# haan6/fm-for-online-recommendation

Measured on AMD Instinct MI355X. Metric: samples/sec online-FM (Criteo-39-field, k=16) FTRL-proximal, higher is better.
Workload: dtype f32

## Files before the change

fm-for-online-recommendation_amd/csrc/fmx_common.h:

```cpp
#pragma once
#include <hip/hip_runtime.h>
#include <hip/hip_ext.h>

#include <cstdarg>
#include <cstdio>
#include <cstdlib>
#include <cstring>
#include <atomic>
#include <mutex>

#include "fmx.h"

#pragma clang fp contract(off)

namespace fmxd {
extern thread_local char g_err[512];
int fail(int code, const char *fmt, ...);
int check_launch(const char *what);

struct Tune {
  int wpb_fwd = 2, wpb_upd = 2;
  int sort_e = 0;
  int inline_fixup = 1;
  int online_persistent = 1;
  int sort_ahead = 16;
  int mlp_chain = 1;
  int sort_chunked = 1;
};
Tune &tune();

constexpr int FMX_COMM_SLOTS = 4;
struct Comm {
  int rank = 0, world = 1, n_blocks = 1;
  bool force = false;
  int block_count[FMX_COMM_MAX_WORLD] = {0}, block_first[FMX_COMM_MAX_WORLD] = {0};
  void *main = nullptr, *pf = nullptr;
  hipStream_t pf_stream = nullptr;
  hipEvent_t fork = nullptr, ready[FMX_COMM_SLOTS] = {nullptr}, free_[FMX_COMM_SLOTS] = {nullptr};
  bool used[FMX_COMM_SLOTS] = {false};
};
int comm_all_gather(Comm *c, int which, const void *send, void *recv, size_t count, hipStream_t st);
int comm_exchange_blocks(Comm *c, const float *send, float *recv, size_t per, hipStream_t st);

constexpr int MLP_BIG_MAX_L = 8;
struct MlpReduceArgs {
  const float *parts[MLP_BIG_MAX_L];
  int out_dim[MLP_BIG_MAX_L], in_dim[MLP_BIG_MAX_L], ldp[MLP_BIG_MAX_L];
  long long grad_off[MLP_BIG_MAX_L];
  float *grads;
  float *params;
  float lr;
  int rule;
  float *m, *v;
  float eps, c1, c2;
  int n_split[MLP_BIG_MAX_L], n_layers;
  const float *loss_b;
  float *loss_out;
  int B;
  float inv_b;
};
int mlp_section_deferred_reduce(const fmx_mlp_t *mlp, int32_t loss_kind, const float *bi, int32_t ld_bi, const float *base, const float *y, int32_t B,
                                float inv_b, void *workspace, float *logit_out, float *dz_out, float *gbi_out, int32_t ld_gbi, float *grads,
                                float lr_apply, float *loss_out, hipStream_t st, MlpReduceArgs *deferred, const char *who = "fmx_mlp_section");
void mlp_launch_reduce(const MlpReduceArgs &a, hipStream_t st);
int mlp_opt_check(const fmx_mlp_t *mlp, int32_t B, const void *workspace, int64_t workspace_bytes, const float *grads, const fmx_mlp_opt_t *opt,
                  int64_t n_steps, const char *who);
int mlp_opt_state_check(const fmx_mlp_opt_t *opt, int64_t n_steps, const char *who);
int mlp_reduce_blocks_per_layer(const MlpReduceArgs &a, int threads);
int step_geometry_check(const fmx_table_t *table, int32_t B, const char *who);
}
using namespace fmxd;

namespace {

inline bool aligned16(const void *p) { return (reinterpret_cast<uintptr_t>(p) & 15u) == 0; }

constexpr uint32_t SENT = 0xFFFFFFFFu;
constexpr int WAVE = 64;
constexpr int MAX_SORT_WIDTH = 32768;


__device__ __forceinline__ float4 operator+(float4 a, float4 b) { return {a.x + b.x, a.y + b.y, a.z + b.z, a.w + b.w}; }
__device__ __forceinline__ float4 operator-(float4 a, float4 b) { return {a.x - b.x, a.y - b.y, a.z - b.z, a.w - b.w}; }
__device__ __forceinline__ float4 operator*(float4 a, float4 b) { return {a.x * b.x, a.y * b.y, a.z * b.z, a.w * b.w}; }
__device__ __forceinline__ float4 operator*(float a, float4 b) { return {a * b.x, a * b.y, a * b.z, a * b.w}; }
__device__ __forceinline__ float4 splat(float a) { return {a, a, a, a}; }

__device__ __forceinline__ float4 shfl_xor4(float4 v, int m) {
  return {__shfl_xor(v.x, m), __shfl_xor(v.y, m), __shfl_xor(v.z, m), __shfl_xor(v.w, m)};
}
__device__ __forceinline__ float4 shfl_up4(float4 v, int d) {
  return {__shfl_up(v.x, d), __shfl_up(v.y, d), __shfl_up(v.z, d), __shfl_up(v.w, d)};
}
__device__ __forceinline__ float4 shfl4(float4 v, int src) {
  return {__shfl(v.x, src), __shfl(v.y, src), __shfl(v.z, src), __shfl(v.w, src)};
}

__device__ __forceinline__ float rcp_(float x) { return __builtin_amdgcn_rcpf(x); }
__device__ __forceinline__ float sqrt_(float x) { return __builtin_amdgcn_sqrtf(x); }

__device__ __forceinline__ float ftrl_w(float z, float n, const fmx_hyper_t &h) {
  const float denom = fmaf(h.beta + sqrt_(n), h.alpha, h.l2);
  const float w = -(z - copysignf(h.l1, z)) * rcp_(denom);
  return fabsf(z) <= h.l1 ? 0.f : w;
}
__device__ __forceinline__ float4 ftrl_w4(float4 z, float4 n, const fmx_hyper_t &h) {
  return {ftrl_w(z.x, n.x, h), ftrl_w(z.y, n.y, h), ftrl_w(z.z, n.z, h), ftrl_w(z.w, n.w, h)};
}
__device__ __forceinline__ void ftrl_upd(float &z, float &n, float w, float g, const fmx_hyper_t &h) {
  const float n2 = fmaf(g, g, n);
  const float sigma = (sqrt_(n2) - sqrt_(n)) * h.alpha;
  z = fmaf(-sigma, w, z + g);
  n = n2;
}

template <int RULE>
__device__ __forceinline__ float apply_rule(float p, float g, const fmx_hyper_t &h) {
  if (RULE == FMX_RULE_SIGNADAM) return p - h.lr * g * rcp_(fabsf(g) + h.eps);
  return p - h.lr * g;
}
template <int RULE>
__device__ __forceinline__ float4 apply_rule4(float4 p, float4 g, const fmx_hyper_t &h) {
  return {apply_rule<RULE>(p.x, g.x, h), apply_rule<RULE>(p.y, g.y, h), apply_rule<RULE>(p.z, g.z, h),
          apply_rule<RULE>(p.w, g.w, h)};
}

__host__ __device__ inline double pow_step(double b, int32_t t) {
  double r = 1.0, p = b;
  for (uint32_t e = (uint32_t)t; e; e >>= 1) {
    if (e & 1u) r = r * p;
    p = p * p;
  }
  return r;
}
__host__ __device__ inline void adam_consts(float lr, float beta1, float beta2, int32_t t, float &step_size, float &c1, float &c2,
                                            float eps = 0.f, float *eps_dense = nullptr) {
  const double b1 = beta1, b2 = beta2;
  const double s2 = sqrt(1.0 - pow_step(b2, t));
  step_size = (float)((double)lr * s2 / (1.0 - pow_step(b1, t)));
  c1 = (float)(1.0 - b1);
  c2 = (float)(1.0 - b2);
  if (eps_dense) *eps_dense = (float)((double)eps * s2);
}
template <int RULE>
__device__ __forceinline__ void moments_upd(float &p, float &m, float &v, float g, const fmx_hyper_t &h) {
  if (RULE == FMX_RULE_ADAM) {
    m = m + h.beta1 * (g - m);
    v = v + h.beta2 * (g * g - v);
    p = p - h.lr * (m * rcp_(sqrt_(v) + h.eps));
  } else {
    v = v + g * g;
    p = p - h.lr * (g * rcp_(sqrt_(v) + h.eps));
  }
}
template <int RULE>
__device__ __forceinline__ void moments_upd4(float4 &p, float4 &m, float4 &v, float4 g, const fmx_hyper_t &h) {
  moments_upd<RULE>(p.x, m.x, v.x, g.x, h);
  moments_upd<RULE>(p.y, m.y, v.y, g.y, h);
  moments_upd<RULE>(p.z, m.z, v.z, g.z, h);
  moments_upd<RULE>(p.w, m.w, v.w, g.w, h);
}

template <int LAYOUT>
__device__ __forceinline__ float bias_weight(float b0, float b1, const fmx_hyper_t &h) {
  return LAYOUT == FMX_LAYOUT_FTRL ? ftrl_w(b0, b1, h) : b0;
}
template <int LAYOUT, int RULE>
__device__ __forceinline__ void bias_step(float &b0, float &b1, float &b2, float g, const fmx_hyper_t &h) {
  if (LAYOUT == FMX_LAYOUT_WEIGHTS) {
    b0 = apply_rule<RULE>(b0, g, h);
  } else if (LAYOUT == FMX_LAYOUT_MOMENTS) {
    moments_upd<RULE>(b0, b1, b2, g, h);
  } else {
    const float w = ftrl_w(b0, b1, h);
    ftrl_upd(b0, b1, w, g, h);
  }
}

__device__ __forceinline__ float sigmoidf_(float z) { return 1.f / (1.f + expf(-z)); }
__device__ __forceinline__ float bcewl(float z, float y) {
  return (1.f - y) * z + log1pf(expf(-fabsf(z))) + fmaxf(-z, 0.f);
}
__device__ __forceinline__ void bce_loss_dz(int loss_kind, float z, float y, float inv_b, float &loss, float &dz) {
  if (loss_kind == FMX_LOSS_BCE_LOGITS) {
    loss = bcewl(z, y);
    dz = (sigmoidf_(z) - y) * inv_b;
  } else {
    const float p = sigmoidf_(z);
    loss = bcewl(p, y);
    dz = (sigmoidf_(p) - y) * p * (1.f - p) * inv_b;
  }
}

template <int M>
__device__ __forceinline__ uint32_t xor_lane(uint32_t v, int lane) {
  if constexpr (M == 1) {
    return (uint32_t)__builtin_amdgcn_mov_dpp((int)v, 0xB1, 0xF, 0xF, true);
  } else if constexpr (M == 2) {
    return (uint32_t)__builtin_amdgcn_mov_dpp((int)v, 0x4E, 0xF, 0xF, true);
  } else if constexpr (M == 4) {
    const int t = __builtin_amdgcn_mov_dpp((int)v, 0x141, 0xF, 0xF, true);
    return (uint32_t)__builtin_amdgcn_mov_dpp(t, 0x1B, 0xF, 0xF, true);
  } else if constexpr (M == 8) {
    return (uint32_t)__builtin_amdgcn_mov_dpp((int)v, 0x128, 0xF, 0xF, true);
  } else if constexpr (M == 16) {
    const auto sw = __builtin_amdgcn_permlane16_swap(v, v, false, false);
    return (lane & 16) ? sw[0] : sw[1];
  } else {
    const auto sw = __builtin_amdgcn_permlane32_swap(v, v, false, false);
    return (lane & 32) ? sw[0] : sw[1];
  }
}

template <int M>
__device__ __forceinline__ float xor_lane_f(float v, int lane) {
  return __uint_as_float(xor_lane<M>(__float_as_uint(v), lane));
}
template <int M>
__device__ __forceinline__ float4 xor_lane_f4(float4 v, int lane) {
  return {xor_lane_f<M>(v.x, lane), xor_lane_f<M>(v.y, lane), xor_lane_f<M>(v.z, lane), xor_lane_f<M>(v.w, lane)};
}

template <int M, int LPR>
__device__ __forceinline__ void fm_sums_level(float4 &s, float4 &ss, float &fo, int lane, int groups) {
  if (LPR <= M && M / LPR < groups) {
    s = s + xor_lane_f4<M>(s, lane);
    ss = ss + xor_lane_f4<M>(ss, lane);
    fo += xor_lane_f<M>(fo, lane);
  }
}
template <int LPR>
__device__ __forceinline__ void fm_field_sums(float4 &s, float4 &ss, float &fo, int lane, int groups = WAVE) {
  fm_sums_level<1, LPR>(s, ss, fo, lane, groups);
  fm_sums_level<2, LPR>(s, ss, fo, lane, groups);
  fm_sums_level<4, LPR>(s, ss, fo, lane, groups);
  fm_sums_level<8, LPR>(s, ss, fo, lane, groups);
  fm_sums_level<16, LPR>(s, ss, fo, lane, groups);
  fm_sums_level<32, LPR>(s, ss, fo, lane, groups);
}
template <int LPR>
__device__ __forceinline__ float4 fm_bi(float4 s, float4 ss, float &sbi) {
  const float4 bi = 0.5f * (s * s - ss);
  sbi = (bi.x + bi.y) + (bi.z + bi.w);
#pragma unroll
  for (int m = 1; m < LPR; m <<= 1) sbi += __shfl_xor(sbi, m);
  return bi;
}

__device__ float block_sum(const float *src, int n, int ld, float *sm) {
  constexpr int U = 16;
  const int tid = threadIdx.x, nt = blockDim.x < 128 ? blockDim.x : 128;
  float acc = 0.f;
  if (tid >= nt) {
    __syncthreads();
    for (int w = nt >> 1; w > 0; w >>= 1) __syncthreads();
    const float r = sm[0];
    __syncthreads();
    return r;
  }
  if (ld == 1) {
    const int n4 = n >> 2;
    const float4 *src4 = reinterpret_cast<const float4 *>(src);
    for (int i0 = tid; i0 < n4; i0 += U * nt) {
      float4 v[U];
#pragma unroll
      for (int u = 0; u < U; ++u) {
        const int i = i0 + u * nt;
        v[u] = src4[i < n4 ? i : 0];
      }
#pragma unroll
      for (int u = 0; u < U; ++u) {
        const bool in = i0 + u * nt < n4;
        acc += in ? (v[u].x + v[u].y) + (v[u].z + v[u].w) : 0.f;
      }
    }
    for (int i = (n4 << 2) + tid; i < n; i += nt) acc += src[i];
  } else {
    constexpr int V = 4;
    const int n4 = n >> 2;
    for (int i0 = tid; i0 < n4; i0 += V * nt) {
      float4 v[V];
#pragma unroll
      for (int u = 0; u < V; ++u) {
        const int i = i0 + u * nt;
        const float *p = src + (size_t)(4 * (i < n4 ? i : 0)) * ld;
        v[u] = float4{p[0], p[ld], p[2 * (size_t)ld], p[3 * (size_t)ld]};
      }
#pragma unroll
      for (int u = 0; u < V; ++u) {
        const bool in = i0 + u * nt < n4;
        acc += in ? (v[u].x + v[u].y) + (v[u].z + v[u].w) : 0.f;
      }
    }
    for (int i = (n4 << 2) + tid; i < n; i += nt) acc += src[(size_t)i * ld];
  }
  sm[tid] = acc;
  __syncthreads();
  for (int w = nt >> 1; w > 0; w >>= 1) {
    if (tid < w) sm[tid] += sm[tid + w];
    __syncthreads();
  }
  const float r = sm[0];
  __syncthreads();
  return r;
}

inline size_t align_up(size_t x, size_t a) { return (x + a - 1) / a * a; }

inline void mlp_reduce_set_opt(MlpReduceArgs &a, const fmx_mlp_opt_t &o, int32_t t) {
  a.rule = o.rule;
  a.m = o.m;
  a.v = o.v;
  a.lr = o.lr;
  a.eps = o.eps;
  a.c1 = a.c2 = 0.f;
  if (o.rule == FMX_RULE_ADAM) adam_consts(o.lr, o.beta1, o.beta2, t, a.lr, a.c1, a.c2, o.eps, &a.eps);
}

__device__ __forceinline__ void mlp_reduce_block(const MlpReduceArgs &a, int l, int block, int n_blocks) {
  const int out = a.out_dim[l], in = a.in_dim[l], ldp = a.ldp[l], ns = a.n_split[l];
  const int groups = ldp >> 2;
  const long long n = (long long)out * groups;
  const float *p = a.parts[l];
  const size_t zs = (size_t)out * ldp;
  const bool adaptive = a.rule != FMX_RULE_SGD, apply = adaptive || a.lr != 0.f;
  fmx_hyper_t h;
  h.lr = a.lr;
  h.eps = a.eps;
  h.beta1 = a.c1;
  h.beta2 = a.c2;
  for (long long i = (long long)block * blockDim.x + threadIdx.x; i < n; i += (long long)n_blocks * blockDim.x) {
    const int m = (int)(i / groups), c = (int)(i - (long long)m * groups) * 4;
    const float *q = p + (size_t)m * ldp + c;
    const bool vec4 = apply && c + 3 < in && (in & 3) == 0 && (a.grad_off[l] & 3) == 0;
    float4 pv = {0.f, 0.f, 0.f, 0.f}, mv = pv, vv = pv;
    if (vec4) {
      const long long o = a.grad_off[l] + (long long)m * in + c;
      pv = *reinterpret_cast<const float4 *>(a.params + o);
      if (adaptive) vv = *reinterpret_cast<const float4 *>(a.v + o);
      if (a.rule == FMX_RULE_ADAM) mv = *reinterpret_cast<const float4 *>(a.m + o);
    }
    float4 s = {0.f, 0.f, 0.f, 0.f};
    for (int z0 = 0; z0 < ns; z0 += 16) {
      float4 r[16];
#pragma unroll
      for (int z = 0; z < 16; ++z)
        if (z0 + z < ns) r[z] = *reinterpret_cast<const float4 *>(q + (size_t)(z0 + z) * zs);
#pragma unroll
      for (int z = 0; z < 16; ++z)
        if (z0 + z < ns) {
          s.x += r[z].x;
          s.y += r[z].y;
          s.z += r[z].z;
          s.w += r[z].w;
        }
    }
    if (vec4) {
      const long long o = a.grad_off[l] + (long long)m * in + c;
      *reinterpret_cast<float4 *>(a.grads + o) = s;
      if (a.rule == FMX_RULE_ADAM) {
        moments_upd4<FMX_RULE_ADAM>(pv, mv, vv, s, h);
        *reinterpret_cast<float4 *>(a.m + o) = mv;
        *reinterpret_cast<float4 *>(a.v + o) = vv;
      } else if (adaptive) {
        moments_upd4<FMX_RULE_ADAGRAD>(pv, mv, vv, s, h);
        *reinterpret_cast<float4 *>(a.v + o) = vv;
      } else {
        pv = float4{pv.x - a.lr * s.x, pv.y - a.lr * s.y, pv.z - a.lr * s.z, pv.w - a.lr * s.w};
      }
      *reinterpret_cast<float4 *>(a.params + o) = pv;
      continue;
    }
    const float v[4] = {s.x, s.y, s.z, s.w};
#pragma unroll
    for (int j = 0; j < 4; ++j) {
      if (c + j > in) break;
      const long long o = c + j < in ? a.grad_off[l] + (long long)m * in + c + j : a.grad_off[l] + (long long)out * in + m;
      a.grads[o] = v[j];
      if (!apply) continue;
      if (!adaptive) {
        a.params[o] -= a.lr * v[j];
      } else if (a.rule == FMX_RULE_ADAM) {
        moments_upd<FMX_RULE_ADAM>(a.params[o], a.m[o], a.v[o], v[j], h);
      } else {
        float unused = 0.f;
        moments_upd<FMX_RULE_ADAGRAD>(a.params[o], unused, a.v[o], v[j], h);
      }
    }
  }
  if (block == 0 && l == 0 && a.loss_out) {
    __shared__ float sm[256];
    const float ls = block_sum(a.loss_b, a.B, 1, sm);
    if (threadIdx.x == 0) a.loss_out[0] = ls * a.inv_b;
  }
}

}
```

fm-for-online-recommendation_amd/csrc/fmx_kernels.hip:

```cpp

#include <type_traits>

#include "fmx_common.h"

namespace fmxd {

thread_local char g_err[512] = "";

int fail(int code, const char *fmt, ...) {
  va_list ap;
  va_start(ap, fmt);
  vsnprintf(g_err, sizeof(g_err), fmt, ap);
  va_end(ap);
  return code;
}

int check_launch(const char *what) {
  hipError_t e = hipGetLastError();
  if (e != hipSuccess) return fail(FMX_ERR_LAUNCH, "%s: %s", what, hipGetErrorString(e));
  return FMX_OK;
}

}

namespace {

#include "fmx_sort.inc"

__device__ __forceinline__ void st_sc1(float *p, float v) { __hip_atomic_store(p, v, __ATOMIC_RELAXED, __HIP_MEMORY_SCOPE_AGENT); }
__device__ __forceinline__ float ld_sc1(const float *p) {
  return __hip_atomic_load(p, __ATOMIC_RELAXED, __HIP_MEMORY_SCOPE_AGENT);
}
__device__ __forceinline__ float4 ld_sc1_4(const float *p) { return {ld_sc1(p), ld_sc1(p + 1), ld_sc1(p + 2), ld_sc1(p + 3)}; }
typedef float v4f __attribute__((ext_vector_type(4)));
__device__ __forceinline__ void st_sc1_4(float *p, float4 v) {
  const v4f x = {v.x, v.y, v.z, v.w};
  asm volatile("global_store_dwordx4 %0, %1, off sc1\n\ts_nop 1" ::"v"(p), "v"(x) : "memory");
}
__device__ __forceinline__ void store_part_sc1(float *rec, int q, int kp, float4 cV, float4 cA, float cw) {
  st_sc1_4(rec + 4 * q, cV);
  st_sc1_4(rec + kp + 4 * q, cA);
  if (q == 0) st_sc1(rec + 2 * kp, cw);
}

struct FwdArgs {
  const float *rows;
  const int64_t *foff;
  const float *bias;
  const int32_t *idx;
  const float *xv;
  const float *y;
  fmx_fwd_out_t out;
  fmx_hyper_t h;
  int32_t B, F, kp, stride, zoff, loss_kind;
  int32_t ldS, ld1;
  float inv_b;
  const int32_t *fcols, *fbase;
  int32_t Fc;
};

#ifdef FMX_STAMPS
__device__ unsigned long long g_fwd_stamps[8192 * 6];
#define FMX_FSTAMP(slot_, dep_)                                                                                     \
  do {                                                                                                              \
    unsigned long long t_;                                                                                          \
    asm volatile("s_memrealtime %0\n\ts_waitcnt lgkmcnt(0)" : "=s"(t_) : "v"(dep_) : "memory");                      \
    if (lane == 0 && b < 8192) g_fwd_stamps[(size_t)b * 6 + (slot_)] = t_;                                           \
  } while (0)
#else
#define FMX_FSTAMP(slot_, dep_) do {} while (0)
#endif

template <int LPR>
__device__ __forceinline__ void forward_finish(const FwdArgs &a, const int b, const int lane, float4 s, float4 ss, float fo, bool bad,
                                               const float y_early, const float bias) {
  const int q = lane % LPR;
  const int kp = LPR * 4;
  if (bad && a.out.error) *a.out.error = 1;

  fm_field_sums<LPR>(s, ss, fo, lane);
  float sbi;
  const float4 bi = fm_bi<LPR>(s, ss, sbi);
  fo = __shfl(fo, 0);
  FMX_FSTAMP(3, sbi);

  if (lane < LPR) {
    if (a.out.S) *reinterpret_cast<float4 *>(a.out.S + (size_t)b * a.ldS + 4 * q) = s;
    if (a.out.bi) *reinterpret_cast<float4 *>(a.out.bi + (size_t)b * kp + 4 * q) = bi;
  }
  if (lane == 0) {
    const float z = fo + sbi + bias;
    if (a.out.sfirst) a.out.sfirst[b] = fo;
    if (a.out.sbi) a.out.sbi[b] = sbi;
    if (a.out.logit) a.out.logit[b] = z;
    if (a.loss_kind != FMX_LOSS_NONE) {
      float loss, dz;
      bce_loss_dz(a.loss_kind, z, y_early, a.inv_b, loss, dz);
      FMX_FSTAMP(4, dz);
      if (a.out.loss) a.out.loss[(size_t)b * a.ld1] = loss;
      if (a.out.dz) a.out.dz[(size_t)b * a.ld1] = dz;
    }
    FMX_FSTAMP(5, z);
  }
}

__device__ __forceinline__ int64_t shfl64(int64_t v, int src) {
  const int lo = __shfl((int)(uint32_t)v, src), hi = __shfl((int)(v >> 32), src);
  return (int64_t)(((uint64_t)(uint32_t)hi << 32) | (uint32_t)lo);
}
constexpr int64_t ROW_ABSENT = int64_t(1) << 62;

template <int LPR, int LAYOUT, int NPASS, bool MAPPED, bool HAS_X>
__device__ __forceinline__ void forward_sample(const FwdArgs &a, const int b, const int lane) {
  constexpr int SLOTS = WAVE / LPR;
  constexpr int NP = NPASS > 0 ? NPASS : 1;
  constexpr int NW = NPASS > 0 ? (NP * SLOTS + WAVE - 1) / WAVE : 1;
  const int slot = lane / LPR, q = lane % LPR;
  const int kp = LPR * 4;
  FMX_FSTAMP(0, lane);

  float4 s = splat(0.f), ss = splat(0.f);
  float fo = 0.f;
  bool bad = false;
  const float y_early = a.loss_kind != FMX_LOSS_NONE ? a.y[b] : 0.f;
  const float bias0_early = a.bias[0];
  const float bias1_early = LAYOUT == FMX_LAYOUT_WEIGHTS ? 0.f : a.bias[1];
  __builtin_amdgcn_sched_barrier(0);
  float bias = 0.f;
  const int n_outer = NPASS > 0 ? 1 : (a.F + SLOTS - 1) / SLOTS;
  for (int it = 0; it < n_outer; ++it) {
    int fl[NW];
    bool wlive[NW];
    int64_t lo[NW], hi[NW];
    uint32_t li[NW];
    float xl[NW];
#pragma unroll
    for (int w = 0; w < NW; ++w) {
      const int f = (NPASS > 0 ? w * WAVE : it * SLOTS) + lane;
      wlive[w] = f < a.F;
      fl[w] = wlive[w] ? f : a.F - 1;
    }
#pragma unroll
    for (int w = 0; w < NW; ++w) {
      lo[w] = a.foff[fl[w]];
      hi[w] = a.foff[fl[w] + 1];
    }
#pragma unroll
    for (int w = 0; w < NW; ++w) {
      size_t o = (size_t)b * a.F + fl[w];
      uint32_t fb = 0u;
      if (MAPPED) {
        o = (size_t)b * a.Fc + (a.fcols ? a.fcols[fl[w]] : fl[w]);
        fb = a.fbase ? (uint32_t)a.fbase[fl[w]] : 0u;
      }
      li[w] = (uint32_t)a.idx[o] - fb;
      xl[w] = HAS_X ? a.xv[o] : 1.f;
    }
    int64_t row[NW];
#pragma unroll
    for (int w = 0; w < NW; ++w) {
      const bool okw = wlive[w] && li[w] < (uint32_t)(hi[w] - lo[w]);
      row[w] = lo[w] + (okw ? li[w] : 0u);
      if (!okw) row[w] |= ROW_ABSENT;
      bad = bad || (!MAPPED && wlive[w] && !okw);
    }
    FMX_FSTAMP(1, (uint32_t)row[0]);
    float x[NP];
    float4 r0[NP];
    float rw[NP];
    bool ok[NP], live[NP];
#pragma unroll
    for (int p = 0; p < NP; ++p) {
      const int f = NPASS > 0 ? p * SLOTS + slot : slot;
      const int w = NPASS > 0 ? (p * SLOTS) / WAVE : 0;
      live[p] = (NPASS > 0 ? f : it * SLOTS + f) < a.F;
      const int64_t r = shfl64(row[w], f % WAVE);
      x[p] = HAS_X ? __shfl(xl[w], f % WAVE) : 1.f;
      ok[p] = live[p] && !(r & ROW_ABSENT);
      const float *rp = a.rows + (size_t)(r & ~ROW_ABSENT) * a.stride;
      r0[p] = *reinterpret_cast<const float4 *>(rp + 4 * q);
      rw[p] = rp[kp];
    }
    __builtin_amdgcn_sched_barrier(0);
    if (it == 0) {
      bias = bias_weight<LAYOUT>(bias0_early, bias1_early, a.h);
      asm volatile("" ::"v"(bias));
    }
    __builtin_amdgcn_sched_barrier(0);
#pragma unroll
    for (int p = 0; p < NP; ++p) {
      const float4 e = x[p] * r0[p];
      const float f1 = ok[p] ? rw[p] * x[p] : 0.f;
      if (ok[p]) {
        s = s + e;
        ss = ss + e * e;
        fo += f1;
      }
      if (live[p] && a.out.first && q == 0) a.out.first[(size_t)b * a.F + (it * NP + p) * SLOTS + slot] = f1;
    }
    FMX_FSTAMP(2, s.x + ss.x + fo);
  }
  forward_finish<LPR>(a, b, lane, s, ss, fo, bad, y_early, bias);
}

template <int LPR, int LAYOUT, int NPASS, bool MAPPED = false>
__global__ __launch_bounds__(256) void k_fm_forward(FwdArgs a) {
  __builtin_amdgcn_s_setprio(3);
  const int b = blockIdx.x * (blockDim.x >> 6) + (threadIdx.x >> 6);
  if (b >= a.B) return;
  if (a.xv) forward_sample<LPR, LAYOUT, NPASS, MAPPED, true>(a, b, threadIdx.x & 63);
  else forward_sample<LPR, LAYOUT, NPASS, MAPPED, false>(a, b, threadIdx.x & 63);
}

struct PartArgs {
  const float *rows;
  const int64_t *foff;
  const int32_t *fcols, *fbase;
  const int32_t *idx;
  const float *xv;
  float *rec;
  int32_t *error;
  int32_t B, F, Fc, stride, sl_log2, group;
};

template <int LPR, int NPASS>
__global__ __launch_bounds__(256) void k_fm_forward_part(PartArgs a) {
  constexpr int SLOTS = WAVE / LPR;
  constexpr int kp = LPR * 4, REC = 2 * kp + 4;
  const int lane = threadIdx.x & 63;
  const int slot = lane / LPR, q = lane % LPR;
  const int SL = 1 << a.sl_log2;
  const int slot_l = slot & (SL - 1);
  const int wave = blockIdx.x * (blockDim.x >> 6) + (threadIdx.x >> 6);
  const int b = wave * (SLOTS >> a.sl_log2) + (slot >> a.sl_log2);
  const bool valid = b < a.B;
  const int f0 = (int)blockIdx.y * NPASS * SL;
  const bool pieces = a.fcols || a.fbase;
  uint32_t li[NPASS], vocab[NPASS];
  float x[NPASS], xl[NPASS];
  int64_t lo[NPASS], hi[NPASS];
  bool live[NPASS], ok[NPASS];
  int fc[NPASS];
  const float *xsrc = a.xv ? a.xv : reinterpret_cast<const float *>(a.idx);
  const bool has_x = a.xv != nullptr;
  const int bc = valid ? b : 0;
#pragma unroll
  for (int p = 0; p < NPASS; ++p) {
    const int f = f0 + p * SL + slot_l;
    live[p] = valid && f < a.F;
    fc[p] = f < a.F ? f : a.F - 1;
  }
  int colp[NPASS];
  uint32_t fb[NPASS];
#pragma unroll
  for (int p = 0; p < NPASS; ++p) {
    lo[p] = a.foff[fc[p]];
    hi[p] = a.foff[fc[p] + 1];
    colp[p] = a.fcols ? a.fcols[fc[p]] : fc[p];
    fb[p] = a.fbase ? (uint32_t)a.fbase[fc[p]] : 0u;
  }
#pragma unroll
  for (int p = 0; p < NPASS; ++p) {
    const size_t o = (size_t)bc * a.Fc + colp[p];
    li[p] = (uint32_t)a.idx[o] - fb[p];
    xl[p] = xsrc[o];
  }
#pragma unroll
  for (int p = 0; p < NPASS; ++p) {
    x[p] = has_x ? xl[p] : 1.f;
    vocab[p] = (uint32_t)(hi[p] - lo[p]);
  }
  float4 r0[NPASS];
  float rw[NPASS];
#pragma unroll
  for (int p = 0; p < NPASS; ++p) {
    ok[p] = live[p] && li[p] < vocab[p];
    const float *rp = a.rows + (size_t)(lo[p] + (ok[p] ? li[p] : 0u)) * a.stride;
    r0[p] = *reinterpret_cast<const float4 *>(rp + 4 * q);
    rw[p] = rp[kp];
  }
  __builtin_amdgcn_sched_barrier(0);
  float4 s = splat(0.f), ss = splat(0.f);
  float fo = 0.f;
  bool bad = false;
#pragma unroll
  for (int p = 0; p < NPASS; ++p) {
    const float4 e = x[p] * r0[p];
    if (ok[p]) {
      s = s + e;
      ss = ss + e * e;
      fo += rw[p] * x[p];
    }
    bad = bad || (!pieces && live[p] && !ok[p]);
  }
  if (bad && a.error) *a.error = 1;
  fm_field_sums<LPR>(s, ss, fo, lane, SL);
  if (valid && slot_l == 0) {
    const int dst = b / a.group;
    float *r = a.rec + (((size_t)dst * gridDim.y + blockIdx.y) * a.group + (b - dst * a.group)) * REC;
    *reinterpret_cast<float4 *>(r + 4 * q) = s;
    *reinterpret_cast<float4 *>(r + kp + 4 * q) = ss;
    if (q == 0) *reinterpret_cast<float4 *>(r + 2 * kp) = float4{fo, 0.f, 0.f, 0.f};
  }
}

struct FinishArgs {
  const float *parts;
  int64_t rank_stride;
  const float *bias;
  const float *y;
  fmx_fwd_out_t out;
  fmx_hyper_t h;
  int32_t B, loss_kind, ldS, ld1;
  float inv_b;
};

template <int LPR, int LAYOUT, int G>
__global__ __launch_bounds__(256) void k_fm_forward_finish(FinishArgs a) {
  constexpr int SLOTS = WAVE / LPR;
  constexpr int kp = LPR * 4, REC = 2 * kp + 4;
  const int lane = threadIdx.x & 63;
  const int slot = lane / LPR, q = lane % LPR;
  const int b = (blockIdx.x * (blockDim.x >> 6) + (threadIdx.x >> 6)) * SLOTS + slot;
  const bool valid = b < a.B;
  const float y_early = (valid && a.loss_kind != FMX_LOSS_NONE) ? a.y[b] : 0.f;
  const float bias0 = a.bias[0];
  const float bias1 = LAYOUT == FMX_LAYOUT_WEIGHTS ? 0.f : a.bias[1];
  float4 s[G], ss[G];
  float fo[G];
#pragma unroll
  for (int r = 0; r < G; ++r) {
    s[r] = ss[r] = splat(0.f);
    fo[r] = 0.f;
    if (valid) {
      const float *p = a.parts + (size_t)r * a.rank_stride + (size_t)b * REC;
      s[r] = *reinterpret_cast<const float4 *>(p + 4 * q);
      ss[r] = *reinterpret_cast<const float4 *>(p + kp + 4 * q);
      if (q == 0) fo[r] = p[2 * kp];
    }
  }
#pragma unroll
  for (int st = 1; st < G; st <<= 1) {
#pragma unroll
    for (int r = 0; r < G; r += 2 * st) {
      s[r] = s[r] + s[r + st];
      ss[r] = ss[r] + ss[r + st];
      fo[r] += fo[r + st];
    }
  }
  float sbi;
  const float4 bi = fm_bi<LPR>(s[0], ss[0], sbi);
  if (!valid) return;
  if (a.out.S) *reinterpret_cast<float4 *>(a.out.S + (size_t)b * a.ldS + 4 * q) = s[0];
  if (a.out.bi) *reinterpret_cast<float4 *>(a.out.bi + (size_t)b * kp + 4 * q) = bi;
  if (q == 0) {
    const float z = fo[0] + sbi + bias_weight<LAYOUT>(bias0, bias1, a.h);
    if (a.out.sfirst) a.out.sfirst[b] = fo[0];
    if (a.out.sbi) a.out.sbi[b] = sbi;
    if (a.out.logit) a.out.logit[b] = z;
    if (a.loss_kind != FMX_LOSS_NONE) {
      float loss, dz;
      bce_loss_dz(a.loss_kind, z, y_early, a.inv_b, loss, dz);
      if (a.out.loss) a.out.loss[(size_t)b * a.ld1] = loss;
      if (a.out.dz) a.out.dz[(size_t)b * a.ld1] = dz;
// ... 1140 lines not shown
  if ((v.x + v.y) + (v.z + v.w) == 123456.789f) *sink = v.x;
}


int lpr_of(int kp) {
  switch (kp) {
    case 4: return 1;
    case 8: return 2;
    case 16: return 4;
    case 32: return 8;
    case 64: return 16;
    default: return 0;
  }
}

template <class Fn>
decltype(auto) with_lpr(int kp, Fn &&f) {
  switch (lpr_of(kp)) {
    case 1: return f(std::integral_constant<int, 1>{});
    case 2: return f(std::integral_constant<int, 2>{});
    case 4: return f(std::integral_constant<int, 4>{});
    case 8: return f(std::integral_constant<int, 8>{});
    default: return f(std::integral_constant<int, 16>{});
  }
}

template <int... VS, class Fn>
bool with_one_of(int v, Fn &&f) {
  return ((v == VS && (f(std::integral_constant<int, VS>{}), true)) || ...);
}

template <bool MOMENTS_RULES, class Fn>
bool with_rule_impl(int rule, Fn &&f) {
  using Weights = std::integral_constant<int, FMX_LAYOUT_WEIGHTS>;
  using Moments = std::integral_constant<int, FMX_LAYOUT_MOMENTS>;
  switch (rule) {
    case FMX_RULE_SIGNADAM: f(Weights{}, std::integral_constant<int, FMX_RULE_SIGNADAM>{}); return true;
    case FMX_RULE_SGD: f(Weights{}, std::integral_constant<int, FMX_RULE_SGD>{}); return true;
    case FMX_RULE_FTRL: f(std::integral_constant<int, FMX_LAYOUT_FTRL>{}, std::integral_constant<int, FMX_RULE_FTRL>{}); return true;
    case FMX_RULE_ADAGRAD:
      if constexpr (MOMENTS_RULES) {
        f(Moments{}, std::integral_constant<int, FMX_RULE_ADAGRAD>{});
        return true;
      }
      return false;
    case FMX_RULE_ADAM:
      if constexpr (MOMENTS_RULES) {
        f(Moments{}, std::integral_constant<int, FMX_RULE_ADAM>{});
        return true;
      }
      return false;
    default: return false;
  }
}
template <class Fn>
bool with_rule(int rule, Fn &&f) { return with_rule_impl<true>(rule, f); }
template <class Fn>
bool with_rule_wf(int rule, Fn &&f) { return with_rule_impl<false>(rule, f); }

inline bool adaptive_rule(int rule) { return rule == FMX_RULE_ADAGRAD || rule == FMX_RULE_ADAM; }
inline const char *rule_name(int rule) { return rule == FMX_RULE_ADAM ? "FMX_RULE_ADAM" : "FMX_RULE_ADAGRAD"; }
int refuse_adaptive(int rule, const char *who) {
  return fail(FMX_ERR_UNSUPPORTED, "%s: %s is not supported here (fmx_fm_update / fmx_fm_step / fmx_fm_stream / fmx_fm_online_run take it)",
              who, rule_name(rule));
}

int check_table(const fmx_table_t *t) {
  if (!t) return fail(FMX_ERR_ARG, "table is null");
  if (!t->rows || !t->field_offsets || !t->bias) return fail(FMX_ERR_ARG, "table has a null pointer");
  if (t->n_fields < 1 || t->n_rows < 1 || t->k < 1) return fail(FMX_ERR_ARG, "table sizes must be positive");
  if (!lpr_of(t->kp) || t->k > t->kp) return fail(FMX_ERR_SHAPE, "kp=%d must be 4/8/16/32/64 and >= k=%d", t->kp, t->k);
  if (t->layout != FMX_LAYOUT_WEIGHTS && t->layout != FMX_LAYOUT_FTRL && t->layout != FMX_LAYOUT_MOMENTS)
    return fail(FMX_ERR_ARG, "unknown layout %d", t->layout);
  int need = t->kp + 4;
  if (t->layout != FMX_LAYOUT_WEIGHTS) {
    if (t->z_offset % 4 || t->z_offset < t->kp + 4)
      return fail(FMX_ERR_SHAPE, "z_offset=%d must be a multiple of 4 and >= kp + 4 = %d", t->z_offset, t->kp + 4);
    need = t->z_offset + 2 * t->kp;
  }
  if (t->row_stride % 4 || t->row_stride < need)
    return fail(FMX_ERR_SHAPE, "row_stride=%d must be a multiple of 4 and >= %d", t->row_stride, need);
  if (!aligned16(t->rows)) return fail(FMX_ERR_ALIGN, "table rows must be 16-byte aligned");
  if (t->max_field_rows < 1 || t->max_field_rows > t->n_rows) return fail(FMX_ERR_SHAPE, "max_field_rows out of range");
  if (t->n_sort_fields < 0 || (t->n_sort_fields > 0 && (t->n_sort_fields < t->n_fields || !t->sort_offsets || !t->sort_cols ||
                                                        t->max_sort_field_rows < 1 || t->max_sort_field_rows > t->max_field_rows)))
    return fail(FMX_ERR_SHAPE, "sort fields: n_sort_fields >= n_fields with sort_offsets, sort_cols and max_sort_field_rows, or 0");
  if (t->n_cols < 0 || (t->field_cols && t->n_cols < 1)) return fail(FMX_ERR_SHAPE, "field_cols needs n_cols >= 1");
  return FMX_OK;
}

int check_rule(const fmx_table_t *t, int rule) {
  if (rule == FMX_RULE_FTRL) {
    if (t->layout != FMX_LAYOUT_FTRL) return fail(FMX_ERR_ARG, "FMX_RULE_FTRL needs FMX_LAYOUT_FTRL");
  } else if (rule == FMX_RULE_SIGNADAM || rule == FMX_RULE_SGD) {
    if (t->layout != FMX_LAYOUT_WEIGHTS) return fail(FMX_ERR_ARG, "rule %d needs FMX_LAYOUT_WEIGHTS", rule);
  } else if (adaptive_rule(rule)) {
    if (t->layout != FMX_LAYOUT_MOMENTS) return fail(FMX_ERR_ARG, "%s needs FMX_LAYOUT_MOMENTS", rule_name(rule));
  } else {
    return fail(FMX_ERR_ARG, "unknown rule %d", rule);
  }
  return FMX_OK;
}

int check_adam(const fmx_hyper_t *h, int rule, int64_t n_steps) {
  if (rule != FMX_RULE_ADAM || !h) return FMX_OK;
  if (!(h->beta1 >= 0.f && h->beta1 < 1.f && h->beta2 >= 0.f && h->beta2 < 1.f))
    return fail(FMX_ERR_ARG, "FMX_RULE_ADAM: beta1 = %g and beta2 = %g must lie in [0, 1)", h->beta1, h->beta2);
  if (h->step < 0 || (int64_t)h->step + n_steps > INT32_MAX)
    return fail(FMX_ERR_ARG, "FMX_RULE_ADAM: step = %d must be >= 0 and step + steps of the call <= 2^31 - 1", h->step);
  return FMX_OK;
}

inline bool mapped(const fmx_table_t *t) { return t->field_cols || t->field_base; }
inline int n_cols(const fmx_table_t *t) { return t->n_cols > 0 ? t->n_cols : t->n_fields; }
inline int n_sort_fields(const fmx_table_t *t) { return t->n_sort_fields > 0 ? t->n_sort_fields : t->n_fields; }
inline const int64_t *sort_offsets(const fmx_table_t *t) { return t->n_sort_fields > 0 ? t->sort_offsets : t->field_offsets; }
inline const int32_t *sort_cols(const fmx_table_t *t) { return t->n_sort_fields > 0 ? t->sort_cols : nullptr; }
inline int64_t max_sort_rows(const fmx_table_t *t) { return t->n_sort_fields > 0 ? t->max_sort_field_rows : t->max_field_rows; }

int check_sort_geometry(const fmx_table_t *t, int B) {
  if (B < 1) return fail(FMX_ERR_ARG, "B must be >= 1");
  const int Bp = fmx_sorted_width(B);
  if (Bp > MAX_SORT_WIDTH)
    return fail(FMX_ERR_UNSUPPORTED, "batch %d exceeds the LDS sort width %d", B, MAX_SORT_WIDTH);
  const int bbits = fmx_sorted_bbits(B);
  if ((uint64_t)(max_sort_rows(t) - 1) >= (uint64_t)(SENT >> bbits))
    return fail(FMX_ERR_UNSUPPORTED, "largest sort field (%lld rows) and batch %d do not fit a 32-bit (index, sample) composite: "
                "split the large fields (fmx_table_t.sort_offsets)", (long long)max_sort_rows(t), B);
  return FMX_OK;
}

}
namespace fmxd {
int step_geometry_check(const fmx_table_t *table, int32_t B, const char *who) {
  int rc = check_table(table);
  if (rc == FMX_OK) rc = check_sort_geometry(table, B);
  if (rc == FMX_OK) return rc;
  char msg[sizeof(g_err)];
  snprintf(msg, sizeof(msg), "%s", g_err);
  return fail(rc, "%s: %s", who, msg);
}
Tune &tune() {
  static Tune t = [] {
    Tune x;
    if (const char *e = getenv("FMX_WPB_FWD")) x.wpb_fwd = atoi(e);
    if (const char *e = getenv("FMX_WPB_UPD")) x.wpb_upd = atoi(e);
    if (const char *e = getenv("FMX_SORT_E")) x.sort_e = atoi(e);
    if (const char *e = getenv("FMX_SORT_AHEAD")) x.sort_ahead = atoi(e);
    if (const char *e = getenv("FMX_ONLINE_PERSISTENT")) x.online_persistent = atoi(e);
    if (const char *e = getenv("FMX_INLINE_FIXUP")) x.inline_fixup = atoi(e);
    if (const char *e = getenv("FMX_SORT_CHUNKED")) x.sort_chunked = atoi(e);
    if (const char *e = getenv("FMX_MLP_CHAIN")) x.mlp_chain = atoi(e);
    auto ok = [](int v) { return v == 1 || v == 2 || v == 4; };
    if (!ok(x.wpb_fwd)) x.wpb_fwd = 2;
    if (!ok(x.wpb_upd)) x.wpb_upd = 2;
    return x;
  }();
  return t;
}
}
namespace {

constexpr int SORT_AHEAD_MAX = 16;

struct Workspace {
  uint32_t *sorted;
  size_t sorted_stride;
  uint32_t *runs;
  int32_t *meta;
  int32_t *counter;
  float *parts;
  size_t bytes;
};



Workspace carve(const fmx_table_t *t, int B, void *base) {
  const size_t F = (size_t)n_sort_fields(t), Bp = (size_t)fmx_sorted_width(B), tiles = Bp >> 6;
  const size_t rec = 2 * (size_t)t->kp + 4;
  const size_t o_sorted1 = align_up(F * Bp * 4, 256);
  const size_t o_runs = 2 * SORT_AHEAD_MAX * o_sorted1;
  const size_t o_meta = o_runs + (Bp >= 2 * SORT_CHUNK ? SORT_AHEAD_MAX * o_sorted1 : 0);
  const size_t o_counter = o_meta + align_up(F * tiles * 2 * 4, 256);
  const size_t o_parts = o_counter + 256;
  Workspace w;
  char *p = static_cast<char *>(base);
  w.sorted = reinterpret_cast<uint32_t *>(p);
  w.sorted_stride = o_sorted1 / 4;
  w.runs = reinterpret_cast<uint32_t *>(p + o_runs);
  w.meta = reinterpret_cast<int32_t *>(p + o_meta);
  w.counter = reinterpret_cast<int32_t *>(p + o_counter);
  w.parts = reinterpret_cast<float *>(p + o_parts);
  w.bytes = o_parts + align_up(F * tiles * 2 * rec * 4, 256);
  return w;
}

int check_workspace(const fmx_table_t *t, int B, const void *workspace, int64_t workspace_bytes, const char *who) {
  if (!workspace) return fail(FMX_ERR_ARG, "%s: null workspace", who);
  if (!aligned16(workspace)) return fail(FMX_ERR_ALIGN, "%s: workspace must be 16-byte aligned", who);
  const int64_t need = (int64_t)carve(t, B, nullptr).bytes;
  if (workspace_bytes < need)
    return fail(FMX_ERR_SHAPE, "%s: workspace of %lld bytes, %lld needed for B = %d and %d sort fields (fmx_workspace_bytes)", who,
                (long long)workspace_bytes, (long long)need, B, n_sort_fields(t));
  return FMX_OK;
}

struct Side {
  hipStream_t stream = nullptr;
  hipStream_t main = nullptr;
  hipEvent_t fork = nullptr, sorted[2] = {nullptr, nullptr}, consumed[2] = {nullptr, nullptr};
  hipEvent_t user_fork = nullptr, user_join = nullptr;
};

Side *side_for_current_device() {
  static std::mutex mu;
  static Side sides[64];
  int dev = 0;
  if (hipGetDevice(&dev) != hipSuccess || dev < 0 || dev >= 64) return nullptr;
  std::lock_guard<std::mutex> lock(mu);
  Side &sd = sides[dev];
  if (!sd.stream) {
    int lo = 0, hi = 0;
    (void)hipDeviceGetStreamPriorityRange(&lo, &hi);
    if (hipStreamCreateWithPriority(&sd.stream, hipStreamNonBlocking, lo) != hipSuccess) return nullptr;
    if (hipStreamCreateWithPriority(&sd.main, hipStreamNonBlocking, hi) != hipSuccess) return nullptr;
    bool ok = hipEventCreateWithFlags(&sd.fork, hipEventDisableTiming) == hipSuccess &&
              hipEventCreateWithFlags(&sd.user_fork, hipEventDisableTiming) == hipSuccess &&
              hipEventCreateWithFlags(&sd.user_join, hipEventDisableTiming) == hipSuccess;
    for (int i = 0; i < 2 && ok; ++i) {
      ok = hipEventCreateWithFlags(&sd.sorted[i], hipEventDisableTiming) == hipSuccess &&
           hipEventCreateWithFlags(&sd.consumed[i], hipEventDisableTiming) == hipSuccess;
    }
    if (!ok) return nullptr;
  }
  return &sd;
}

constexpr int OVERLAP_MIN_BATCH = 512;

template <int LPR, int NPASS, bool MAPPED = false>
void launch_forward_np(const FwdArgs &a, int layout, hipStream_t st) {
  const int wpb = tune().wpb_fwd;
  const dim3 grid((a.B + wpb - 1) / wpb), block(64 * wpb);
  if (layout == FMX_LAYOUT_FTRL) hipLaunchKernelGGL((k_fm_forward<LPR, FMX_LAYOUT_FTRL, NPASS, MAPPED>), grid, block, 0, st, a);
  else hipLaunchKernelGGL((k_fm_forward<LPR, FMX_LAYOUT_WEIGHTS, NPASS, MAPPED>), grid, block, 0, st, a);
}

template <int LPR>
void launch_forward(const FwdArgs &a, int layout, hipStream_t st) {
  const int slots = WAVE / LPR;
  const int np = (a.F + slots - 1) / slots;
  if (a.fcols || a.fbase)
    launch_forward_np<LPR, 0, true>(a, layout, st);
  else if (!with_one_of<1, 2, 3, 4>(np, [&](auto NP) { launch_forward_np<LPR, NP>(a, layout, st); }))
    launch_forward_np<LPR, 0>(a, layout, st);
}

bool is_capturing(hipStream_t st) {
  if (!st) return false;
  hipStreamCaptureStatus cs = hipStreamCaptureStatusNone;
  return hipStreamIsCapturing(st, &cs) == hipSuccess && cs != hipStreamCaptureStatusNone;
}

template <int LPR, bool HAS_GBI, bool INL>
void launch_update(const UpdArgs &a, int rule, hipStream_t st) {
  const int tiles = a.F * (a.Bp >> 6);
  const int wpb = tune().wpb_upd;
  const dim3 grid((tiles + wpb - 1) / wpb + red_slices(a.B)), block(64 * wpb);
  with_rule(rule, [&](auto LAYOUT, auto RULE) { hipLaunchKernelGGL((k_fm_update<LPR, LAYOUT, RULE, HAS_GBI, INL>), grid, block, 0, st, a); });
}

template <int LPR>
void launch_update_rider(const UpdArgs &a, int rule, const MlpReduceArgs &r, hipStream_t st) {
  const int tiles = a.F * (a.Bp >> 6);
  const int wpb = tune().wpb_upd;
  const int n_upd = (tiles + wpb - 1) / wpb + red_slices(a.B), per = mlp_reduce_blocks_per_layer(r, 64 * wpb);
  const dim3 grid(n_upd + per * r.n_layers), block(64 * wpb);
  with_rule(rule, [&](auto LAYOUT, auto RULE) {
    hipLaunchKernelGGL((k_fm_update_rider<LPR, LAYOUT, RULE, true>), grid, block, 0, st, a, r, n_upd, per);
  });
}

template <int LPR>
void launch_fixup(const UpdArgs &a, int rule, hipStream_t st) {
  const int tiles = a.F * (a.Bp >> 6);
  const int wpb = tune().wpb_upd;
  const dim3 grid((tiles + wpb - 1) / wpb + (red_slices(a.B) > 1 ? 1 : 0)), block(64 * wpb);
  with_rule(rule, [&](auto LAYOUT, auto RULE) { hipLaunchKernelGGL((k_fm_fixup<LPR, LAYOUT, RULE>), grid, block, 0, st, a); });
}

template <int LPR>
void launch_update_pair(const UpdArgs &a, int rule, bool has_gbi, hipStream_t st) {
  if (tune().inline_fixup && !is_capturing(st)) {
    if (has_gbi) launch_update<LPR, true, true>(a, rule, st);
    else launch_update<LPR, false, true>(a, rule, st);
    return;
  }
  if (has_gbi) launch_update<LPR, true, false>(a, rule, st);
  else launch_update<LPR, false, false>(a, rule, st);
  launch_fixup<LPR>(a, rule, st);
}

template <int LPR>
void launch_update_occ_pair(const UpdArgs &a, int rule, hipStream_t st) {
  const int tiles = a.F * (a.Bp >> 6);
  const int wpb = tune().wpb_upd;
  const dim3 grid((tiles + wpb - 1) / wpb + red_slices(a.B)), block(64 * wpb);
// ... 1126 lines not shown
```

Baseline: 191.9 million.

## Gather per-sample loss tail into first wave and use DPP reductions in forward

Raises the default forward block from 2 to 4 waves. When a loss is computed, each wave's scalar results (first-order sum, pairwise term, label) go into shared memory after a block barrier, and wave 0 computes logit, loss and dz for all samples in the block with one lane per sample, instead of one lane per wave. The pairwise-term lane reduction now uses DPP xor-lane ops, and readfirstlane replaces a shuffle. Out-of-range waves stay alive with a clamped index so they can reach the barrier, which adds a block-wide sync and some redundant loads in exchange for fewer serialized scalar tails.

```diff
diff --git a/fm-for-online-recommendation_amd/csrc/fmx_common.h b/fm-for-online-recommendation_amd/csrc/fmx_common.h
--- a/fm-for-online-recommendation_amd/csrc/fmx_common.h
+++ b/fm-for-online-recommendation_amd/csrc/fmx_common.h
@@ -19,7 +19,7 @@
 int check_launch(const char *what);
 
 struct Tune {
-  int wpb_fwd = 2, wpb_upd = 2;
+  int wpb_fwd = 4, wpb_upd = 2;
   int sort_e = 0;
   int inline_fixup = 1;
   int online_persistent = 1;
@@ -246,6 +246,16 @@
   for (int m = 1; m < LPR; m <<= 1) sbi += __shfl_xor(sbi, m);
   return bi;
 }
+template <int LPR>
+__device__ __forceinline__ float4 fm_bi_dpp(float4 s, float4 ss, float &sbi) {
+  const float4 bi = 0.5f * (s * s - ss);
+  sbi = (bi.x + bi.y) + (bi.z + bi.w);
+  if (LPR > 1) sbi += xor_lane_f<1>(sbi, 0);
+  if (LPR > 2) sbi += xor_lane_f<2>(sbi, 0);
+  if (LPR > 4) sbi += xor_lane_f<4>(sbi, 0);
+  if (LPR > 8) sbi += xor_lane_f<8>(sbi, 0);
+  return bi;
+}
 
 __device__ float block_sum(const float *src, int n, int ld, float *sm) {
   constexpr int U = 16;
diff --git a/fm-for-online-recommendation_amd/csrc/fmx_kernels.hip b/fm-for-online-recommendation_amd/csrc/fmx_kernels.hip
--- a/fm-for-online-recommendation_amd/csrc/fmx_kernels.hip
+++ b/fm-for-online-recommendation_amd/csrc/fmx_kernels.hip
@@ -61,46 +61,68 @@
 
 #ifdef FMX_STAMPS
 __device__ unsigned long long g_fwd_stamps[8192 * 6];
-#define FMX_FSTAMP(slot_, dep_)                                                                                     \
+#define FMX_FSTAMP_AT(slot_, dep_, first_, count_)                                                                  \
   do {                                                                                                              \
     unsigned long long t_;                                                                                          \
     asm volatile("s_memrealtime %0\n\ts_waitcnt lgkmcnt(0)" : "=s"(t_) : "v"(dep_) : "memory");                      \
-    if (lane == 0 && b < 8192) g_fwd_stamps[(size_t)b * 6 + (slot_)] = t_;                                           \
+    if (lane < (count_) && (first_) + lane < 8192) g_fwd_stamps[(size_t)((first_) + lane) * 6 + (slot_)] = t_;       \
   } while (0)
 #else
-#define FMX_FSTAMP(slot_, dep_) do {} while (0)
+#define FMX_FSTAMP_AT(slot_, dep_, first_, count_) do {} while (0)
 #endif
+#define FMX_FSTAMP(slot_, dep_) FMX_FSTAMP_AT(slot_, dep_, b, (int)exists)
+
+__device__ __forceinline__ float first_lane_f(float v) { return __int_as_float(__builtin_amdgcn_readfirstlane(__float_as_int(v))); }
 
 template <int LPR>
-__device__ __forceinline__ void forward_finish(const FwdArgs &a, const int b, const int lane, float4 s, float4 ss, float fo, bool bad,
-                                               const float y_early, const float bias) {
+__device__ __forceinline__ void forward_finish(const FwdArgs &a, int b, const bool exists, const int lane, float4 s, float4 ss, float fo,
+                                               bool bad, float y, const float bias) {
   const int q = lane % LPR;
   const int kp = LPR * 4;
   if (bad && a.out.error) *a.out.error = 1;
 
   fm_field_sums<LPR>(s, ss, fo, lane);
   float sbi;
-  const float4 bi = fm_bi<LPR>(s, ss, sbi);
-  fo = __shfl(fo, 0);
+  const float4 bi = fm_bi_dpp<LPR>(s, ss, sbi);
+  fo = first_lane_f(fo);
   FMX_FSTAMP(3, sbi);
 
-  if (lane < LPR) {
+  if (exists && lane < LPR) {
     if (a.out.S) *reinterpret_cast<float4 *>(a.out.S + (size_t)b * a.ldS + 4 * q) = s;
     if (a.out.bi) *reinterpret_cast<float4 *>(a.out.bi + (size_t)b * kp + 4 * q) = bi;
   }
-  if (lane == 0) {
+  int n = exists ? 1 : 0;
+  if (a.loss_kind != FMX_LOSS_NONE && blockDim.x > WAVE) {
+    __shared__ float sh[3][4];
+    const int w = threadIdx.x >> 6, wpb = blockDim.x >> 6;
+    if (lane == 0) {
+      sh[0][w] = fo;
+      sh[1][w] = sbi;
+      sh[2][w] = y;
+    }
+    __syncthreads();
+    if (w != 0) return;
+    b = blockIdx.x * wpb;
+    n = min(wpb, a.B - b);
+    const int l = lane < n ? lane : 0;
+    fo = sh[0][l];
+    sbi = sh[1][l];
+    y = sh[2][l];
+  }
+  if (lane < n) {
+    const int bl = b + lane;
     const float z = fo + sbi + bias;
-    if (a.out.sfirst) a.out.sfirst[b] = fo;
-    if (a.out.sbi) a.out.sbi[b] = sbi;
-    if (a.out.logit) a.out.logit[b] = z;
+    if (a.out.sfirst) a.out.sfirst[bl] = fo;
+    if (a.out.sbi) a.out.sbi[bl] = sbi;
+    if (a.out.logit) a.out.logit[bl] = z;
     if (a.loss_kind != FMX_LOSS_NONE) {
       float loss, dz;
-      bce_loss_dz(a.loss_kind, z, y_early, a.inv_b, loss, dz);
-      FMX_FSTAMP(4, dz);
-      if (a.out.loss) a.out.loss[(size_t)b * a.ld1] = loss;
-      if (a.out.dz) a.out.dz[(size_t)b * a.ld1] = dz;
-    }
-    FMX_FSTAMP(5, z);
+      bce_loss_dz(a.loss_kind, z, y, a.inv_b, loss, dz);
+      FMX_FSTAMP_AT(4, dz, b, n);
+      if (a.out.loss) a.out.loss[(size_t)bl * a.ld1] = loss;
+      if (a.out.dz) a.out.dz[(size_t)bl * a.ld1] = dz;
+    }
+    FMX_FSTAMP_AT(5, z, b, n);
   }
 }
 
@@ -111,7 +133,7 @@
 constexpr int64_t ROW_ABSENT = int64_t(1) << 62;
 
 template <int LPR, int LAYOUT, int NPASS, bool MAPPED, bool HAS_X>
-__device__ __forceinline__ void forward_sample(const FwdArgs &a, const int b, const int lane) {
+__device__ __forceinline__ void forward_sample(const FwdArgs &a, const int b, const bool exists, const int lane) {
   constexpr int SLOTS = WAVE / LPR;
   constexpr int NP = NPASS > 0 ? NPASS : 1;
   constexpr int NW = NPASS > 0 ? (NP * SLOTS + WAVE - 1) / WAVE : 1;
@@ -196,20 +218,21 @@
         ss = ss + e * e;
         fo += f1;
       }
-      if (live[p] && a.out.first && q == 0) a.out.first[(size_t)b * a.F + (it * NP + p) * SLOTS + slot] = f1;
+      if (exists && live[p] && a.out.first && q == 0) a.out.first[(size_t)b * a.F + (it * NP + p) * SLOTS + slot] = f1;
     }
     FMX_FSTAMP(2, s.x + ss.x + fo);
   }
-  forward_finish<LPR>(a, b, lane, s, ss, fo, bad, y_early, bias);
+  forward_finish<LPR>(a, b, exists, lane, s, ss, fo, bad, y_early, bias);
 }
 
 template <int LPR, int LAYOUT, int NPASS, bool MAPPED = false>
 __global__ __launch_bounds__(256) void k_fm_forward(FwdArgs a) {
   __builtin_amdgcn_s_setprio(3);
-  const int b = blockIdx.x * (blockDim.x >> 6) + (threadIdx.x >> 6);
-  if (b >= a.B) return;
-  if (a.xv) forward_sample<LPR, LAYOUT, NPASS, MAPPED, true>(a, b, threadIdx.x & 63);
-  else forward_sample<LPR, LAYOUT, NPASS, MAPPED, false>(a, b, threadIdx.x & 63);
+  int b = blockIdx.x * (blockDim.x >> 6) + (threadIdx.x >> 6);
+  const bool exists = b < a.B;
+  if (!exists) b = a.B - 1;
+  if (a.xv) forward_sample<LPR, LAYOUT, NPASS, MAPPED, true>(a, b, exists, threadIdx.x & 63);
+  else forward_sample<LPR, LAYOUT, NPASS, MAPPED, false>(a, b, exists, threadIdx.x & 63);
 }
 
 struct PartArgs {
@@ -1656,7 +1679,7 @@
     if (const char *e = getenv("FMX_SORT_CHUNKED")) x.sort_chunked = atoi(e);
     if (const char *e = getenv("FMX_MLP_CHAIN")) x.mlp_chain = atoi(e);
     auto ok = [](int v) { return v == 1 || v == 2 || v == 4; };
-    if (!ok(x.wpb_fwd)) x.wpb_fwd = 2;
+    if (!ok(x.wpb_fwd)) x.wpb_fwd = 4;
     if (!ok(x.wpb_upd)) x.wpb_upd = 2;
     return x;
   }();
```

Measured after the change: 200.6 million (median of 6 runs). 4.5% higher.
